# jan-van-bergen/GPU-Raytracer

Hardware: AMD Instinct MI355X
Metric: Mrays/s (primary+secondary) + ms/frame, Sponza 1920x1080 4spp BVH8 (higher is better)
Workload: dtype f32

## Files before the change

### gpu-raytracer_amd/csrc/kernels_trace.hip

```cpp
#include "rt_math.h"

#include <cstdio>
#include <cstdlib>

#ifndef RT_LDS_STACK
#define RT_LDS_STACK   10
#endif
#define RT_STACK_SIZE  32
#define RT_TRACE_BLOCK 256
#ifndef RT_TRACE_WAVES_PER_SIMD
#define RT_TRACE_WAVES_PER_SIMD 6
#endif
#ifndef RT_TRI_BATCH
#define RT_TRI_BATCH 2
#endif
#ifndef RT_FETCH_BLOCK_MAX
#define RT_FETCH_BLOCK_MAX 256
#endif
#ifndef RT_ENDGAME
#define RT_ENDGAME 1
#endif
#ifndef RT_ENDGAME_REGION_MAX
#define RT_ENDGAME_REGION_MAX 256
#endif
// ... 297 lines not shown
}

RT_DEV int opacity_wrap(int i, int n) { if ((n & (n - 1)) == 0) return i & (n - 1); int r = i % n; return r < 0 ? r + n : r; }
RT_DEV bool opacity_accepts(const RtParams & p, int instance, int triangle_id, float u, float v) {
	if (p.has_triangle_aliases) {
		float4 names = p.triangle_positions[size_t(triangle_id) * 3 + 2];
		if (__float_as_int(names.z) >= 0) { instance = __float_as_int(names.z); triangle_id = __float_as_int(names.w); }
	}
	int material = p.mesh_material_ids[instance];
	if (material < 0) return true;
	int mask_index = p.material_opacity[material];
	if (mask_index == RT_INVALID) return true;
	RtOpacityMask mask = p.opacity_masks[mask_index];
	const float4 * shading = p.triangles + size_t(triangle_id) * 6;
	float4 a = shading[4], b = shading[5];
	float s = a.z + u * b.x + v * b.z;
	float t = a.w + u * b.y + v * b.w;
	int x = opacity_wrap(int(floorf(s * float(mask.width))),  mask.width);
	int y = opacity_wrap(int(floorf(t * float(mask.height))), mask.height);
	unsigned i = unsigned(y) * unsigned(mask.width) + unsigned(x);
	return (mask.bits[i >> 5] >> (i & 31u)) & 1u;
}

template<bool MASK = false>
RT_DEV bool triangle_test_kind(bool shadow, float4 part_0, float4 part_1, float4 part_2, int mesh_id, int triangle_id, const Ray3 & ray, HitRecord & hit, const RtParams * p = nullptr) {
	f3 p0 = mk3(part_0.x, part_0.y, part_0.z);
	f3 e1 = mk3(part_0.w, part_1.x, part_1.y);
	f3 e2 = mk3(part_1.z, part_1.w, part_2.x);

	f3 h = cross_fma(ray.direction, e2);
	float a = dot_fma(e1, h);
	float f = 1.0f / a;
	f3 s = ray.origin - p0;
	float u = f * dot_fma(s, h);
	if (u >= 0.0f && u <= 1.0f) {
		f3 q = cross_fma(s, e1);
		float v = f * dot_fma(ray.direction, q);
		if (v >= 0.0f && u + v <= 1.0f) {
			float t = f * dot_fma(e2, q);
			if (t > 0.0f && t < hit.t) {
				if (MASK && !opacity_accepts(*p, mesh_id, triangle_id, u, v)) return false;
				if (shadow) return true;
				hit.t = t; hit.u = u; hit.v = v;
				hit.mesh_id = mesh_id;
				hit.triangle_id = triangle_id;
			}
		}
	}
	return false;
}

template<bool SHADOW>
RT_DEV bool triangle_test(const float4 * __restrict__ triangle_positions, int mesh_id, int triangle_id, const Ray3 & ray, float max_distance, HitRecord & hit) {
	const float4 * tri = triangle_positions + size_t(triangle_id) * 3;
	return triangle_test_loaded<SHADOW>(tri[0], tri[1], tri[2], mesh_id, triangle_id, ray, max_distance, hit);
}

typedef __attribute__((address_space(3))) uint2 LdsUint2;
typedef __attribute__((address_space(1))) uint2 GlobalUint2;
struct TraversalStack {
	LdsUint2    * lds;
	GlobalUint2 * spill;
	int spill_stride;
	int size;

	RT_DEV void push(uint2 item) {
		if (size < RT_LDS_STACK) { lds[size * RT_WAVE_SIZE].x = item.x; lds[size * RT_WAVE_SIZE].y = item.y; }
		else { GlobalUint2 * slot = spill + size_t(size - RT_LDS_STACK) * spill_stride; slot->x = item.x; slot->y = item.y; }
		size++;
	}
	RT_DEV uint2 pop() {
		size--;
		if (size < RT_LDS_STACK) return make_uint2(lds[size * RT_WAVE_SIZE].x, lds[size * RT_WAVE_SIZE].y);
		const GlobalUint2 * slot = spill + size_t(size - RT_LDS_STACK) * spill_stride;
		return make_uint2(slot->x, slot->y);
	}
};


__shared__ uint2 shared_stack[(RT_TRACE_BLOCK / RT_WAVE_SIZE) * RT_LDS_STACK * RT_WAVE_SIZE];
__shared__ int   shared_fetch[RT_TRACE_BLOCK / RT_WAVE_SIZE][4];
#define RT_ROOTS_IN_LDS 1024
__shared__ int   shared_roots[RT_ROOTS_IN_LDS];
enum { RT_TRACE_CLOSEST = 0, RT_TRACE_SHADOW = 1, RT_TRACE_MIXED = 2 };
template<int MODE, typename Source> RT_DEV void source_load(const Source & src, bool shadow, int i, Ray3 & ray, float & max_distance) {
	if constexpr (MODE == RT_TRACE_MIXED) src.load(shadow, i, ray, max_distance); else src.load(i, ray, max_distance);
}
template<int MODE, typename Source> RT_DEV void source_finish(const Source & src, bool shadow, int i, const HitRecord & hit, bool occluded) {
	if constexpr (MODE == RT_TRACE_MIXED) src.finish(shadow, i, hit, occluded); else src.finish(i, hit, occluded);
}

template<int MODE, bool COUNT, bool NARROW, bool UNIFIED = false, bool FLAT = false, bool SKIP = false, bool MASK = false, typename Source>
RT_DEV void bvh8_trace_engine(const RtParams & p, Source & src, int ray_count, int * cursor, unsigned long long * stats = nullptr, int ray_count_2 = 0, int * cursor_2 = nullptr, int * regions = nullptr) {
	constexpr bool SHADOW = MODE == RT_TRACE_SHADOW;
	bool lane_shadow = SHADOW;
	#define RT_IS_SHADOW (MODE == RT_TRACE_MIXED ? lane_shadow : SHADOW)
	const float4 * __restrict__ nodes     = p.bvh8_nodes;
	const float4 * __restrict__ triangles = p.triangle_positions;

	unsigned lane = threadIdx.x & (RT_WAVE_SIZE - 1);
	unsigned wave = threadIdx.x / RT_WAVE_SIZE;
	const unsigned group_child = lane & 7u;
	const unsigned group_base  = lane & ~7u;

	TraversalStack stack;
	stack.lds   = (LdsUint2 *)&shared_stack[wave * (RT_LDS_STACK * RT_WAVE_SIZE) + lane];
	stack.spill_stride = int(gridDim.x * blockDim.x);
	stack.spill = (GlobalUint2 *)(p.stack_spill + (blockIdx.x * blockDim.x + threadIdx.x));
	stack.size  = 0;

	const int waves_in_grid = int(gridDim.x) * (RT_TRACE_BLOCK / RT_WAVE_SIZE);
	const int rays_total = ray_count + (MODE == RT_TRACE_MIXED ? ray_count_2 : 0);
	const bool endgame = !NARROW && regions != nullptr && waves_in_grid <= RT_ENDGAME_MAX_WAVES;
	const int ray_block = NARROW ? 8 : endgame ? RT_FETCH_BLOCK_MAX : max(RT_WAVE_SIZE, min(RT_FETCH_BLOCK_MAX, (rays_total / (RT_FETCH_BLOCK_DIVISOR * waves_in_grid)) & ~(RT_WAVE_SIZE - 1)));
	const int region_size  = max(RT_WAVE_SIZE, min(RT_ENDGAME_REGION_MAX, ((rays_total + waves_in_grid - 1) / waves_in_grid + RT_WAVE_SIZE - 1) & ~(RT_WAVE_SIZE - 1)));
	const int region_count = min(waves_in_grid, (rays_total + region_size - 1) / region_size);
	const int main_limit   = endgame ? max(0, rays_total - region_count * region_size) : 0;
	const int region_stride = max(1, region_count / RT_WAVE_SIZE) | 1;
	const unsigned wave_in_grid = blockIdx.x * (RT_TRACE_BLOCK / RT_WAVE_SIZE) + wave;
	if (endgame ? wave_in_grid >= unsigned(region_count) : wave_in_grid * unsigned(ray_block) >= unsigned(rays_total)) return;
	typedef volatile __attribute__((address_space(3))) int LdsFetchWord;
	LdsFetchWord * fetch_state = (LdsFetchWord *)&shared_fetch[wave][0];
	if (lane == 0) { fetch_state[0] = 0; fetch_state[1] = 0; fetch_state[2] = 0; fetch_state[3] = 0; }
	auto fetch_ray = [&]() -> int {
		while (endgame) {
			if (fetch_state[2]) return -1;
			unsigned long long want = __ballot(1);
			int n_want = __popcll(want);
			unsigned rank = __builtin_amdgcn_mbcnt_hi(unsigned(want >> 32), __builtin_amdgcn_mbcnt_lo(unsigned(want), 0u));
			bool elected = rank == 0;
			int next = fetch_state[0], end = fetch_state[1];
			if (next >= end) {
				int region = fetch_state[3];
				if (region == 0) {
					int base = main_limit;
					if (main_limit > 0) { if (elected) base = atomicAdd(cursor, ray_block); base = __builtin_amdgcn_readfirstlane(base); }
					if (base < main_limit) { next = base; end = min(base + ray_block, main_limit); }
					else region = int(wave_in_grid) + 1;
				}
				if (region != 0) {
					next = 0; end = 0;
					int scan_from = region, scanned = 0;
					while (true) {
						int taken = 0;
						if (elected) taken = atomicAdd(&regions[region - 1], RT_WAVE_SIZE);
						taken = __builtin_amdgcn_readfirstlane(taken);
						int first = main_limit + (region - 1) * region_size + taken;
						if (taken < region_size && first < rays_total) { next = first; end = min(first + RT_WAVE_SIZE, rays_total); break; }
						bool found = false;
						while (!found && scanned < RT_ENDGAME_SCAN_LIMIT) {
							int candidate = scan_from + (int(rank) + 1) * region_stride;
							while (candidate >= region_count) candidate -= region_count;
							int seen = __hip_atomic_load(&regions[candidate], __ATOMIC_RELAXED, __HIP_MEMORY_SCOPE_AGENT);
							bool open = seen < region_size && main_limit + candidate * region_size + seen < rays_total;
							unsigned long long open_lanes = __ballot(open);
							if (open_lanes) {
								int lane_of_first = __ffsll((long long)open_lanes) - 1;
								region = __builtin_amdgcn_readlane(candidate, lane_of_first) + 1; found = true;
							} else { scan_from = scan_from + 1 < region_count ? scan_from + 1 : 0; scanned++; }
						}
						if (!found) break;
					}
				}
				if (elected) fetch_state[3] = region;
			}
			int give = min(n_want, end - next);
			if (elected) {
				fetch_state[0] = next + give;
				fetch_state[1] = end;
				if (next >= end) fetch_state[2] = 1;
			}
			if (int(rank) < give) {
				int index = next + int(rank);
				if (MODE == RT_TRACE_MIXED) { lane_shadow = index >= ray_count; if (lane_shadow) index -= ray_count; }
				return index;
			}
		}
		while (true) {
			if (fetch_state[2]) return -1;
			const bool second_queue = MODE == RT_TRACE_MIXED && fetch_state[3] != 0;
			const int queue_count = second_queue ? ray_count_2 : ray_count;
			int * const queue_cursor = second_queue ? cursor_2 : cursor;
			unsigned long long want = __ballot(1);
			unsigned long long askers = NARROW ? (want & 0x0101010101010101ull) : want;
			int n_want = __popcll(askers);
			bool elected = __builtin_amdgcn_mbcnt_hi(unsigned(want >> 32), __builtin_amdgcn_mbcnt_lo(unsigned(want), 0u)) == 0;
			unsigned rank = NARROW ? unsigned(__popcll(askers & ((1ull << group_base) - 1ull)))
			                       : __builtin_amdgcn_mbcnt_hi(unsigned(want >> 32), __builtin_amdgcn_mbcnt_lo(unsigned(want), 0u));
			int next = fetch_state[0], end = fetch_state[1];
			if (next >= end) {
				int base = 0;
				if (elected) base = atomicAdd(queue_cursor, ray_block);
				base = __builtin_amdgcn_readfirstlane(base);
				next = min(base, queue_count);
				end  = min(base + ray_block, queue_count);
			}
			int give = min(n_want, end - next);
			if (elected) {
				fetch_state[0] = next + give;
				fetch_state[1] = end;
				if (next >= end) {
					if (MODE == RT_TRACE_MIXED && !second_queue) { fetch_state[0] = 0; fetch_state[1] = 0; fetch_state[3] = 1; }
					else fetch_state[2] = 1;
				}
			}
			if (int(rank) < give) { if (MODE == RT_TRACE_MIXED) lane_shadow = second_queue; return next + int(rank); }
		}
	};

	uint2 current_group = make_uint2(0, 0);
	uint2 triangle_group = make_uint2(0, 0);

	int  ray_index = 0;
	Ray3 ray;
	f3   inv_dir;
	unsigned oct_inv4 = 0;
	HitRecord hit;
	int  tlas_stack_size = RT_INVALID;
	int  mesh_id = 0;
	bool mesh_has_identity_transform = true;
	unsigned count_nodes = 0, count_triangles = 0, count_inst_xform = 0, count_inst_ident = 0;

	unsigned long long lane_totals[2][5] = { { 0, 0, 0, 0, 0 }, { 0, 0, 0, 0, 0 } };
	auto flush_counts = [&]() {
		#pragma unroll
		for (int kind = 0; kind < (MODE == RT_TRACE_MIXED ? 2 : 1); kind++) {
			#pragma unroll
			for (int k = 0; k < 5; k++) if (lane_totals[kind][k]) atomicAdd(&stats[kind * 5 + k], lane_totals[kind][k]);
		}
	};
	int result_pending = 0;
	while (true) {
		bool inactive = stack.size == 0 && current_group.y == 0 && triangle_group.y == 0;

		if (result_pending) {
			if (!RT_IS_SHADOW && p.has_triangle_aliases && hit.triangle_id != RT_INVALID) {
				float4 names = triangles[size_t(hit.triangle_id) * 3 + 2];
				if (__float_as_int(names.z) >= 0) { hit.mesh_id = __float_as_int(names.z); hit.triangle_id = __float_as_int(names.w); }
			}
			if (!NARROW || group_child == 0) source_finish<MODE>(src, RT_IS_SHADOW, ray_index, hit, result_pending == 2);
			result_pending = 0;
		}
		if (inactive) {
			ray_index = fetch_ray();
			if (ray_index < 0) { if constexpr (COUNT) flush_counts(); return; }

			float max_distance;
			source_load<MODE>(src, RT_IS_SHADOW, ray_index, ray, max_distance);
			inv_dir  = reciprocal(ray.direction);
			oct_inv4 = ray_get_octant_inv4(ray.direction);

			hit.t = max_distance; hit.u = 0.0f; hit.v = 0.0f; hit.mesh_id = 0; hit.triangle_id = RT_INVALID;
			current_group   = make_uint2(0, 0x80000000u);
			tlas_stack_size = FLAT ? 0 : p.entry_tlas_stack_size;
		}

		int iterations_lost = 0;
		bool running = true;
		do {
			if (running) {
			if (!FLAT && triangle_group.y != 0 && tlas_stack_size == RT_INVALID) {
				int mesh_offset = int(msb(triangle_group.y));
				triangle_group.y &= ~(1u << mesh_offset);
				mesh_id = int(triangle_group.x) + mesh_offset;

				if (triangle_group.y != 0)         stack.push(triangle_group);
				if (current_group.y & 0xff000000u) stack.push(current_group);
				tlas_stack_size = stack.size;
				triangle_group.y = 0;

				unsigned root = unsigned(UNIFIED && p.mesh_count <= RT_ROOTS_IN_LDS ? shared_roots[mesh_id] : p.mesh_bvh_root_indices[mesh_id]);
				mesh_has_identity_transform = (root >> 31) != 0;
				if (!mesh_has_identity_transform) {
					const float4 * m = p.mesh_transforms_inv + size_t(mesh_id) * 3;
					ray.origin    = transform_position (m, ray.origin);
					ray.direction = transform_direction(m, ray.direction);
					inv_dir  = reciprocal(ray.direction);
					oct_inv4 = ray_get_octant_inv4(ray.direction);
					if (COUNT) count_inst_xform++;
				} else if (COUNT) count_inst_ident++;
				current_group = make_uint2(root & 0x7fffffffu, 0x80000000u);
			}

			RT_SETPRIO(RT_PHASE_TOP);
			if (triangle_group.y == 0) {
				if (current_group.y & 0xff000000u) {
					unsigned hits_imask = current_group.y;
					unsigned child_index_offset = msb(hits_imask);
					unsigned child_index_base   = current_group.x;

					current_group.y &= ~(1u << child_index_offset);
					if (current_group.y & 0xff000000u) stack.push(current_group);

					unsigned slot_index     = (child_index_offset - 24) ^ (oct_inv4 & 0xffu);
					unsigned relative_index = __popc(hits_imask & ~(0xffffffffu << slot_index));
					unsigned child_node_index = child_index_base + relative_index;

					const float4 * node = FLAT ? (const float4 *)((const char *)nodes + __umul24(child_node_index, 80u))
					                    : (!UNIFIED && child_node_index < unsigned(p.tlas_node_count) ? p.tlas_nodes : nodes) + size_t(child_node_index) * 5;
					float4 n0 = node[0], n1 = node[1], n2 = node[2], n3 = node[3], n4 = node[4];
					RT_SETPRIO(RT_PHASE_NODE_TEST);
					if (COUNT) count_nodes++;
					unsigned hitmask, bound_bits = 0;
					if (NARROW) {
						int key;
						hitmask = group8_or(bvh8_node_intersect_child(ray, inv_dir, oct_inv4, hit.t, n0, n1, n2, n3, n4, group_child, SKIP ? &key : nullptr));
						if (SKIP) {
							int least = group8_min_signed(key);
							int second = group8_min_signed(key == least ? RT_SKIP_NO_KEY : key);
							bound_bits = skip_bound_bits(hitmask, least, second);
						}
					} else if (RT_FAST_NODE && UNIFIED && FLAT) hitmask = bvh8_node_intersect_fast<SKIP>(ray, inv_dir, oct_inv4, hit.t, n0, n1, n2, n3, n4, &bound_bits);
					else hitmask = bvh8_node_intersect<SKIP>(ray, inv_dir, oct_inv4, hit.t, n0, n1, n2, n3, n4, &bound_bits);
					unsigned imask = extract_byte(__float_as_uint(n0.w), 3);

					current_group .x = __float_as_uint(n1.x);
					triangle_group.x = __float_as_uint(n1.y);
					current_group .y = (hitmask & 0xff000000u) | imask | (SKIP ? bound_bits : 0u);
					triangle_group.y = (hitmask & 0x00ffffffu);
				}
			}
			RT_SETPRIO(RT_PHASE_TRI_ADDRESS);

			bool occluded = false;
			{
				bool has_triangles = triangle_group.y != 0 && (FLAT || tlas_stack_size != RT_INVALID);
				if (has_triangles) {
					if (NARROW) {
						unsigned rest = triangle_group.y; int my_bit = -1;
						#pragma unroll
						for (unsigned k = 0; k < 8; k++) {
							if (rest != 0) { int b = int(msb(rest)); if (k == group_child) my_bit = b; rest &= ~(1u << b); }
						}
						triangle_group.y = rest;
						float t = 0.0f, u = 0.0f, v = 0.0f; bool valid = false; int my_triangle = RT_INVALID;
						if (my_bit >= 0) {
							my_triangle = int(triangle_group.x) + my_bit;
							const float4 * tri = triangles + size_t(my_triangle) * 3;
// ... 68 lines not shown
						oct_inv4 = ray_get_octant_inv4(ray.direction);
					}
				}
				current_group = stack.pop();
				if ((current_group.y & 0xff000000u) == 0) {
					triangle_group = current_group;
					current_group  = make_uint2(0, 0);
				}
				}
			}
			if constexpr (COUNT) if (result_pending) {
				const int kind = MODE == RT_TRACE_MIXED && lane_shadow ? 1 : 0;
				lane_totals[kind][0] += count_nodes;      lane_totals[kind][1] += count_triangles;
				lane_totals[kind][2] += count_inst_xform; lane_totals[kind][3] += count_inst_ident;
				lane_totals[kind][4] += 1;
				count_nodes = count_triangles = count_inst_xform = count_inst_ident = 0;
			}
			}

			iterations_lost += RT_WAVE_SIZE - __popcll(__ballot(running)) - RT_N_D;
		} while (iterations_lost < RT_N_W);
	}
	#undef RT_IS_SHADOW
}


#define RT_TRACE_LAUNCH_WAVES RT_TRACE_WAVES_PER_SIMD
#ifndef RT_MIXED_MAX_RAYS
#define RT_MIXED_MAX_RAYS (10 * 1024 * 1024)
#endif
#ifndef RT_NARROW_MAX_RAYS
#define RT_NARROW_MAX_RAYS 16384
#endif

template<bool SHADOW, bool COUNT, bool MASK = false, typename Source>
RT_DEV void bvh8_trace_persistent(const RtParams & p, const Source & src, int ray_count, int * cursor, unsigned long long * stats = nullptr, bool coherent = false) {
	const bool narrow = !COUNT && !coherent && ray_count <= RT_NARROW_MAX_RAYS;
	if (!SHADOW && rt_skip_walk(p)) {
		if (narrow) bvh8_trace_engine<RT_TRACE_CLOSEST, false, true, false, false, true, MASK>(p, src, ray_count, cursor);
		else bvh8_trace_engine<RT_TRACE_CLOSEST, COUNT, false, false, false, true, MASK>(p, src, ray_count, cursor, stats);
		return;
	}
	if (narrow) bvh8_trace_engine<SHADOW ? RT_TRACE_SHADOW : RT_TRACE_CLOSEST, false, true, false, false, false, MASK>(p, src, ray_count, cursor);
	else bvh8_trace_engine<SHADOW ? RT_TRACE_SHADOW : RT_TRACE_CLOSEST, COUNT, false, false, false, false, MASK>(p, src, ray_count, cursor, stats);
}

RT_DEV uint4 pack_hit(const HitRecord & h) {
	unsigned uv = unsigned(int(h.u * 65535.0f)) | (unsigned(int(h.v * 65535.0f)) << 16);
	return make_uint4(unsigned(h.mesh_id), unsigned(h.triangle_id), __float_as_uint(h.t), uv);
}


struct ClosestHitSource {
	RtVec3SoA origin, direction;
	uint4 * hits;
	RT_DEV void load(int i, Ray3 & ray, float & max_distance) const { ray.origin = load3(origin, i); ray.direction = load3(direction, i); max_distance = RT_INFINITY; }
	RT_DEV void finish(int i, const HitRecord & hit, bool) const { hits[i] = pack_hit(hit); }
};

struct ShadowQueueSource {
	RtShadowBuffer buffer;
	RtAOV radiance, direct, indirect;
	int bounce;
	RT_DEV void load(int i, Ray3 & ray, float & max_distance) const { ray.origin = load3(buffer.origin, i); ray.direction = load3(buffer.direction, i); max_distance = buffer.max_distance[i]; }
	RT_DEV void finish(int i, const HitRecord &, bool occluded) const {
		if (occluded) return;
		float4 ip = buffer.illumination_and_pixel_index[i];
		int pixel_index = __float_as_int(ip.w);
		float4 value = make_float4(ip.x, ip.y, ip.z, 0.0f);
		if (radiance.framebuffer) { float4 c = radiance.framebuffer[pixel_index]; radiance.framebuffer[pixel_index] = make_float4(c.x + value.x, c.y + value.y, c.z + value.z, c.w + value.w); }
		if (bounce == 0) {
			if (direct.framebuffer) direct.framebuffer[pixel_index] = value;
		} else if (indirect.framebuffer) {
			float4 c = indirect.framebuffer[pixel_index];
			indirect.framebuffer[pixel_index] = make_float4(c.x + value.x, c.y + value.y, c.z + value.z, c.w + value.w);
		}
	}
};

struct ShadowStreamSource {
	RtShadowBuffer buffer;
	RtAOV radiance, direct, indirect;
	RT_DEV void load(int i, Ray3 & ray, float & max_distance) const { ray.origin = load3(buffer.origin, i); ray.direction = load3(buffer.direction, i); max_distance = buffer.max_distance[i]; }
	RT_DEV void finish(int i, const HitRecord &, bool occluded) const {
		if (occluded) return;
		float4 ip = buffer.illumination_and_pixel_index[i];
		unsigned pixel_word = __float_as_uint(ip.w);
		int pixel_index = int(pixel_word & ~RT_SHADOW_FLAG_BOUNCE_0);
		float4 value = make_float4(ip.x, ip.y, ip.z, 0.0f);
		if (radiance.framebuffer) { float4 c = radiance.framebuffer[pixel_index]; radiance.framebuffer[pixel_index] = make_float4(c.x + value.x, c.y + value.y, c.z + value.z, c.w + value.w); }
		if (pixel_word & RT_SHADOW_FLAG_BOUNCE_0) {
			if (direct.framebuffer) direct.framebuffer[pixel_index] = value;
		} else if (indirect.framebuffer) {
			float4 c = indirect.framebuffer[pixel_index];
			indirect.framebuffer[pixel_index] = make_float4(c.x + value.x, c.y + value.y, c.z + value.z, c.w + value.w);
		}
	}
};

struct ShadowAOSource {
	RtShadowBuffer buffer;
	RtAOV radiance;
	RT_DEV void load(int i, Ray3 & ray, float & max_distance) const { ray.origin = load3(buffer.origin, i); ray.direction = load3(buffer.direction, i); max_distance = buffer.max_distance[i]; }
	RT_DEV void finish(int i, const HitRecord &, bool occluded) const {
		if (occluded || !radiance.framebuffer) return;
		int pixel_index = __float_as_int(buffer.illumination_and_pixel_index[i].w);
		radiance.framebuffer[pixel_index] = make_float4(1.0f, 1.0f, 1.0f, 1.0f);
	}
};

struct ShadowExplicitSource {
	RtVec3SoA origin, direction;
	const float * max_dist;
	uint8_t * occluded_out;
	RT_DEV void load(int i, Ray3 & ray, float & max_distance) const { ray.origin = load3(origin, i); ray.direction = load3(direction, i); max_distance = max_dist[i]; }
	RT_DEV void finish(int i, const HitRecord &, bool occluded) const { occluded_out[i] = occluded ? 1 : 0; }
};



RT_DEV bool aabb_intersect(f3 lo, f3 hi, const Ray3 & ray, f3 inv_dir, float limit, float & t_near) {
	float t0x = (lo.x - ray.origin.x) * inv_dir.x, t1x = (hi.x - ray.origin.x) * inv_dir.x;
	float t0y = (lo.y - ray.origin.y) * inv_dir.y, t1y = (hi.y - ray.origin.y) * inv_dir.y;
	float t0z = (lo.z - ray.origin.z) * inv_dir.z, t1z = (hi.z - ray.origin.z) * inv_dir.z;
	t_near      = fmaxf(fminf(t0x, t1x), fmaxf(fminf(t0y, t1y), fmaxf(fminf(t0z, t1z), 0.0f)));
	float t_far = fminf(fmaxf(t0x, t1x), fminf(fmaxf(t0y, t1y), fminf(fmaxf(t0z, t1z), limit)));
	return t_near < t_far;
}

struct LeafRange { int first, count; };

struct Bvh2Step {
	const float4 * __restrict__ nodes;
	RT_DEV explicit Bvh2Step(const RtParams & p) : nodes(p.bvh2_nodes) {}
	RT_DEV LeafRange step(const RtParams & p, TraversalStack & stack, uint2 entry, Ray3 ray, f3 inv_dir, float limit) const {
		const float4 * node = (entry.x < unsigned(p.tlas_node_count) ? p.tlas_nodes : nodes) + size_t(entry.x) * 2;
		float4 a = node[0], b = node[1];
		int      left_or_first = __float_as_int(b.z);
		unsigned count_axis    = __float_as_uint(b.w);
		unsigned count = count_axis & 0x3fffffffu, axis = count_axis >> 30;
		float t_near;
		if (!aabb_intersect(mk3(a.x, a.y, a.z), mk3(a.w, b.x, b.y), ray, inv_dir, limit, t_near)) return { 0, 0 };
		if (count > 0) return { left_or_first, int(count) };
		float d = axis == 0 ? ray.direction.x : (axis == 1 ? ray.direction.y : ray.direction.z);
		bool left_first = d > 0.0f;
		stack.push(make_uint2(unsigned(left_first ? left_or_first + 1 : left_or_first), 0));
		stack.push(make_uint2(unsigned(left_first ? left_or_first : left_or_first + 1), 0));
		return { 0, 0 };
	}
};

RT_DEV float float4_at(float4 v, int i) { return i == 0 ? v.x : (i == 1 ? v.y : (i == 2 ? v.z : v.w)); }
struct Bvh4Step {
	const float4 * __restrict__ nodes;
	RT_DEV explicit Bvh4Step(const RtParams & p) : nodes(p.bvh4_nodes) {}
	RT_DEV LeafRange step(const RtParams & p, TraversalStack & stack, uint2 entry, Ray3 ray, f3 inv_dir, float limit) const {
		int index = int(entry.x), count = int(entry.y);
		if (count > 0) return { index, count };
		const float4 * node = (index < p.tlas_node_count ? p.tlas_nodes : nodes) + size_t(index) * 8;
		float4 min_x = node[0], min_y = node[1], min_z = node[2], max_x = node[3], max_y = node[4], max_z = node[5], ic01 = node[6], ic23 = node[7];
		float t_near[4]; unsigned hit_mask = 0;
		#pragma unroll
		for (int i = 0; i < 4; i++) {
			float tn;
			if (aabb_intersect(mk3(float4_at(min_x, i), float4_at(min_y, i), float4_at(min_z, i)),
			                   mk3(float4_at(max_x, i), float4_at(max_y, i), float4_at(max_z, i)), ray, inv_dir, limit, tn)) hit_mask |= 1u << i;
			t_near[i] = __uint_as_float((__float_as_uint(tn) & 0xfffffffcu) | unsigned(i));
		}
// ... 90 lines not shown
					if (tri_next < tri_end && !occluded) {
						const float4 * tri = triangles + size_t(tri_next) * 3;
						if (triangle_test_loaded<SHADOW>(tri[0], tri[1], make_float4(tri[2].x, 0.0f, 0.0f, 0.0f), mesh_id, tri_next, ray, max_distance, hit)) occluded = true;
						tri_next++;
					}
				}
			} else {
				if (stack.size == tlas_stack_size) {
					tlas_stack_size = RT_INVALID;
					if (!mesh_has_identity_transform) {
						float unused;
						src.load(ray_index, ray, unused);
						inv_dir = reciprocal(ray.direction);
					}
				}
				uint2 entry = stack.pop();
				LeafRange leaf = node_step.step(p, stack, entry, ray, inv_dir, SHADOW ? max_distance : hit.t);
				if (leaf.count > 0) {
					if (tlas_stack_size == RT_INVALID) {
						tlas_stack_size = stack.size;
						mesh_id = leaf.first;
						unsigned root = unsigned(p.mesh_bvh_root_indices[mesh_id]);
						mesh_has_identity_transform = (root >> 31) != 0;
						if (!mesh_has_identity_transform) {
							const float4 * m = p.mesh_transforms_inv + size_t(mesh_id) * 3;
							ray.origin    = transform_position (m, ray.origin);
							ray.direction = transform_direction(m, ray.direction);
							inv_dir = reciprocal(ray.direction);
						}
						stack.push(make_uint2(root & 0x7fffffffu, 0));
					} else {
						tri_next = leaf.first; tri_end = leaf.first + leaf.count;
					}
				}
			}

			if (SHADOW && occluded) {
				src.finish(ray_index, hit, true);
				stack.size = 0; tri_next = tri_end = 0;
				break;
			}
			if (stack.size == 0 && tri_next >= tri_end) {
				src.finish(ray_index, hit, false);
				break;
			}
			iterations_lost += RT_WAVE_SIZE - __popcll(__ballot(1)) - RT_N_D;
		} while (iterations_lost < RT_N_W);
	}
}

RT_DEV ClosestHitSource  closest_queue(const RtParams & p, int bounce) { return { p.trace[bounce & 1].origin, p.trace[bounce & 1].direction, p.trace[bounce & 1].hits }; }
RT_DEV ShadowQueueSource shadow_queue (const RtParams & p, int bounce) { return { p.shadow, p.aovs[RT_AOV_RADIANCE], p.aovs[RT_AOV_RADIANCE_DIRECT], p.aovs[RT_AOV_RADIANCE_INDIRECT], bounce }; }
RT_DEV ShadowAOSource    ao_queue     (const RtParams & p)             { return { p.shadow, p.aovs[RT_AOV_RADIANCE] }; }

#ifndef RT_MASK_WAVES
#define RT_MASK_WAVES RT_TRACE_LAUNCH_WAVES
#endif
#define RT_BVH8_KERNELS(SUFFIX, WAVES, MASK) \
__global__ void __launch_bounds__(RT_TRACE_BLOCK, WAVES) kernel_trace_bvh8##SUFFIX(RtParams p, int bounce) { bvh8_trace_persistent<false, false, MASK>(p, closest_queue(p, bounce), p.sizes->trace[bounce], p.ray_cursors + 2 * bounce, nullptr, bounce == 0); } \
__global__ void __launch_bounds__(RT_TRACE_BLOCK, WAVES) kernel_trace_shadow_bvh8##SUFFIX(RtParams p, int bounce) { bvh8_trace_persistent<true, false, MASK>(p, shadow_queue(p, bounce), p.sizes->shadow[bounce], p.ray_cursors + 2 * bounce + 1); } \
__global__ void __launch_bounds__(RT_TRACE_BLOCK, WAVES) kernel_trace_shadow_bvh8_ao##SUFFIX(RtParams p) { bvh8_trace_persistent<true, false, MASK>(p, ao_queue(p), p.sizes->shadow[0], p.ray_cursors + 1); } \
__global__ void __launch_bounds__(RT_TRACE_BLOCK, WAVES) kernel_trace_bvh8_counting##SUFFIX(RtParams p, int bounce, unsigned long long * stats) { bvh8_trace_persistent<false, true, MASK>(p, closest_queue(p, bounce), p.sizes->trace[bounce], p.ray_cursors + 2 * bounce, stats); } \
__global__ void __launch_bounds__(RT_TRACE_BLOCK, WAVES) kernel_trace_shadow_bvh8_counting##SUFFIX(RtParams p, int bounce, unsigned long long * stats) { bvh8_trace_persistent<true, true, MASK>(p, shadow_queue(p, bounce), p.sizes->shadow[bounce], p.ray_cursors + 2 * bounce + 1, stats + 5); } \
__global__ void __launch_bounds__(RT_TRACE_BLOCK, WAVES) kernel_trace_bvh8_explicit##SUFFIX(RtParams p, RtVec3SoA origin, RtVec3SoA direction, uint4 * hits, int ray_count, int * retired) { bvh8_trace_persistent<false, false, MASK>(p, ClosestHitSource { origin, direction, hits }, ray_count, retired); } \
__global__ void __launch_bounds__(RT_TRACE_BLOCK, WAVES) kernel_trace_shadow_bvh8_explicit##SUFFIX(RtParams p, RtVec3SoA origin, RtVec3SoA direction, const float * max_distance, uint8_t * occluded, int ray_count, int * retired) { bvh8_trace_persistent<true, false, MASK>(p, ShadowExplicitSource { origin, direction, max_distance, occluded }, ray_count, retired); }
RT_BVH8_KERNELS(, RT_TRACE_LAUNCH_WAVES, false)
RT_BVH8_KERNELS(_mask, RT_MASK_WAVES, true)
#undef RT_BVH8_KERNELS

#define RT_BVH_KERNELS(WIDTH, STEP) \
__global__ void __launch_bounds__(RT_TRACE_BLOCK, RT_TRACE_LAUNCH_WAVES) kernel_trace_##WIDTH(RtParams p, int bounce) { bvh_trace_persistent<STEP, false>(p, closest_queue(p, bounce), p.sizes->trace[bounce], p.ray_cursors + 2 * bounce); } \
__global__ void __launch_bounds__(RT_TRACE_BLOCK, RT_TRACE_LAUNCH_WAVES) kernel_trace_shadow_##WIDTH(RtParams p, int bounce) { bvh_trace_persistent<STEP, true>(p, shadow_queue(p, bounce), p.sizes->shadow[bounce], p.ray_cursors + 2 * bounce + 1); } \
__global__ void __launch_bounds__(RT_TRACE_BLOCK, RT_TRACE_LAUNCH_WAVES) kernel_trace_shadow_##WIDTH##_ao(RtParams p) { bvh_trace_persistent<STEP, true>(p, ao_queue(p), p.sizes->shadow[0], p.ray_cursors + 1); } \
__global__ void __launch_bounds__(RT_TRACE_BLOCK, RT_TRACE_LAUNCH_WAVES) kernel_trace_##WIDTH##_explicit(RtParams p, RtVec3SoA origin, RtVec3SoA direction, uint4 * hits, int ray_count, int * retired) { bvh_trace_persistent<STEP, false>(p, ClosestHitSource { origin, direction, hits }, ray_count, retired); } \
__global__ void __launch_bounds__(RT_TRACE_BLOCK, RT_TRACE_LAUNCH_WAVES) kernel_trace_shadow_##WIDTH##_explicit(RtParams p, RtVec3SoA origin, RtVec3SoA direction, const float * max_distance, uint8_t * occluded, int ray_count, int * retired) { bvh_trace_persistent<STEP, true>(p, ShadowExplicitSource { origin, direction, max_distance, occluded }, ray_count, retired); }
RT_BVH_KERNELS(bvh2, Bvh2Step)
RT_BVH_KERNELS(bvh4, Bvh4Step)
#undef RT_BVH_KERNELS

struct MixedStreamSource {
	ClosestHitSource closest; ShadowStreamSource shadow;
	RT_DEV void load(bool is_shadow, int i, Ray3 & ray, float & max_distance) const { if (is_shadow) shadow.load(i, ray, max_distance); else closest.load(i, ray, max_distance); }
	RT_DEV void finish(bool is_shadow, int i, const HitRecord & hit, bool occluded) const { if (is_shadow) shadow.finish(i, hit, occluded); else closest.finish(i, hit, occluded); }
};
#ifdef RT_WAVE_CLOCK
#define RT_WAVE_CLOCK_SLOTS 32
#define RT_WAVE_CLOCK_WAVES 16384
__device__ unsigned long long grt_wave_clock[RT_WAVE_CLOCK_SLOTS][RT_WAVE_CLOCK_WAVES][3];
__device__ int grt_wave_clock_meta[RT_WAVE_CLOCK_SLOTS][4];
extern "C" int rt_debug_read_wave_clock(void * clocks, void * meta) {
	if (hipMemcpyFromSymbol(clocks, HIP_SYMBOL(grt_wave_clock), sizeof(grt_wave_clock)) != hipSuccess) return 1;
	return hipMemcpyFromSymbol(meta, HIP_SYMBOL(grt_wave_clock_meta), sizeof(grt_wave_clock_meta)) != hipSuccess;
}
template<bool COUNT, bool FLAT = false, bool SKIP = false, bool MASK = false> RT_DEV void trace_stream_probed(const RtParams & p, unsigned long long * stats, unsigned long long * mid);
template<bool COUNT, bool FLAT = false, bool SKIP = false, bool MASK = false>
RT_DEV void trace_stream(const RtParams & p, unsigned long long * stats) {
	const unsigned long long t0 = __builtin_amdgcn_s_memrealtime();
	unsigned long long t1 = 0;
	trace_stream_probed<COUNT, FLAT, SKIP, MASK>(p, stats, &t1);
	const unsigned long long t2 = __builtin_amdgcn_s_memrealtime();
	if ((threadIdx.x & 63) == 0) {
		const int slot = p.stream_iteration % RT_WAVE_CLOCK_SLOTS, wave = blockIdx.x * (RT_TRACE_BLOCK / RT_WAVE_SIZE) + threadIdx.x / RT_WAVE_SIZE;
		if (wave < RT_WAVE_CLOCK_WAVES) { grt_wave_clock[slot][wave][0] = t0; grt_wave_clock[slot][wave][1] = t1 ? t1 : t2; grt_wave_clock[slot][wave][2] = t2; }
		if (wave == 0) { const int q = p.stream_iteration & 1; grt_wave_clock_meta[slot][0] = p.stream_iteration; grt_wave_clock_meta[slot][1] = p.stream->trace_count[q]; grt_wave_clock_meta[slot][2] = p.stream->shadow_count[q ^ 1]; grt_wave_clock_meta[slot][3] = gridDim.x * (RT_TRACE_BLOCK / RT_WAVE_SIZE); }
	}
}
#define trace_stream_body trace_stream_probed
#define RT_WAVE_CLOCK_MID , unsigned long long * mid
#define RT_WAVE_CLOCK_MARK *mid = __builtin_amdgcn_s_memrealtime();
#else
template<bool COUNT, bool FLAT = false, bool SKIP = false, bool MASK = false> RT_DEV void trace_stream(const RtParams & p, unsigned long long * stats);
#define trace_stream_body trace_stream
#define RT_WAVE_CLOCK_MID
#define RT_WAVE_CLOCK_MARK
#endif
template<bool COUNT, bool FLAT, bool SKIP, bool MASK>
RT_DEV void trace_stream_body(const RtParams & p, unsigned long long * stats RT_WAVE_CLOCK_MID) {
	const int q = p.stream_iteration & 1;
	MixedStreamSource src { { p.trace[q].origin, p.trace[q].direction, p.trace[q].hits },
	                        { p.shadow, p.aovs[RT_AOV_RADIANCE], p.aovs[RT_AOV_RADIANCE_DIRECT], p.aovs[RT_AOV_RADIANCE_INDIRECT] } };
	const int closest_count = p.stream->trace_count[q], shadow_count = p.stream->shadow_count[q ^ 1];
	if (!FLAT && p.mesh_count <= RT_ROOTS_IN_LDS) {
		for (int i = threadIdx.x; i < p.mesh_count; i += RT_TRACE_BLOCK) shared_roots[i] = p.mesh_bvh_root_indices[i];
		__syncthreads();
	}
	if (!COUNT && closest_count + shadow_count <= RT_NARROW_MAX_RAYS)
		bvh8_trace_engine<RT_TRACE_MIXED, false, true, true, FLAT, SKIP, MASK>(p, src, closest_count, &p.stream->cursor[q][0], nullptr, shadow_count, &p.stream->cursor[q][1]);
	else if (COUNT || closest_count + shadow_count <= RT_MIXED_MAX_RAYS)
		bvh8_trace_engine<RT_TRACE_MIXED, COUNT, false, true, FLAT, SKIP, MASK>(p, src, closest_count, &p.stream->cursor[q][0], stats, shadow_count, &p.stream->cursor[q][1], RT_ENDGAME ? &p.stream->endgame[q][0][0] : nullptr);
	else {
		bvh8_trace_engine<RT_TRACE_CLOSEST, false, false, true, FLAT, SKIP, MASK>(p, src.closest, closest_count, &p.stream->cursor[q][0], nullptr, 0, nullptr, RT_ENDGAME ? &p.stream->endgame[q][0][0] : nullptr);
		RT_WAVE_CLOCK_MARK
		bvh8_trace_engine<RT_TRACE_SHADOW,  false, false, true, FLAT, false, MASK>(p, src.shadow,  shadow_count,  &p.stream->cursor[q][1], nullptr, 0, nullptr, RT_ENDGAME ? &p.stream->endgame[q][1][0] : nullptr);
	}
}
__global__ void __launch_bounds__(RT_TRACE_BLOCK, RT_TRACE_LAUNCH_WAVES) kernel_trace_stream_bvh8(RtParams p) { trace_stream<false>(p, nullptr); }
#ifndef RT_FLAT_WAVES
#define RT_FLAT_WAVES (RT_FAST_NODE ? 6 : 7)
#endif
__global__ void __launch_bounds__(RT_TRACE_BLOCK, RT_FLAT_WAVES) kernel_trace_stream_bvh8_flat(RtParams p) { trace_stream<false, true>(p, nullptr); }
#ifndef RT_FLAT_SKIP_WAVES
#define RT_FLAT_SKIP_WAVES RT_FLAT_WAVES
#endif
__global__ void __launch_bounds__(RT_TRACE_BLOCK, RT_FLAT_SKIP_WAVES) kernel_trace_stream_bvh8_flat_skip(RtParams p) { trace_stream<false, true, true>(p, nullptr); }
__global__ void __launch_bounds__(RT_TRACE_BLOCK, RT_TRACE_LAUNCH_WAVES) kernel_trace_stream_bvh8_counting(RtParams p, unsigned long long * stats) {
	if (rt_skip_walk(p)) trace_stream<true, false, true>(p, stats); else trace_stream<true>(p, stats);
}
__global__ void __launch_bounds__(RT_TRACE_BLOCK, RT_MASK_WAVES) kernel_trace_stream_bvh8_mask(RtParams p) { trace_stream<false, false, false, true>(p, nullptr); }
__global__ void __launch_bounds__(RT_TRACE_BLOCK, RT_MASK_WAVES) kernel_trace_stream_bvh8_flat_mask(RtParams p) { trace_stream<false, true, false, true>(p, nullptr); }
__global__ void __launch_bounds__(RT_TRACE_BLOCK, RT_MASK_WAVES) kernel_trace_stream_bvh8_flat_skip_mask(RtParams p) { trace_stream<false, true, true, true>(p, nullptr); }
__global__ void __launch_bounds__(RT_TRACE_BLOCK, RT_MASK_WAVES) kernel_trace_stream_bvh8_counting_mask(RtParams p, unsigned long long * stats) {
	if (rt_skip_walk(p)) trace_stream<true, false, true, true>(p, stats); else trace_stream<true, false, false, true>(p, stats);
}

static int trace_grid_size(const void * kernel) {
	static const int cus = [] {
		int device = 0, count = 0;
		(void)hipGetDevice(&device);
		(void)hipDeviceGetAttribute(&count, hipDeviceAttributeMultiprocessorCount, device);
		return count > 0 ? count : 256;
	}();
	int blocks_per_cu = 0;
	if (hipOccupancyMaxActiveBlocksPerMultiprocessor(&blocks_per_cu, kernel, RT_TRACE_BLOCK, 0) != hipSuccess || blocks_per_cu <= 0) blocks_per_cu = 2;
	if (blocks_per_cu > 8) blocks_per_cu = 8;
	return cus * blocks_per_cu;
}

template<auto K> static int persistent_grid() {
	static const int grid = trace_grid_size((const void *)K);
	return grid;
}
template<auto K, typename... A> static void launch_persistent(hipStream_t stream, const A &... args) {
	hipLaunchKernelGGL(K, dim3(persistent_grid<K>()), dim3(RT_TRACE_BLOCK), 0, stream, args...);
}
template<auto K8, auto K8M, typename... A> static void launch_for_mask(const RtParams & p, hipStream_t stream, const A &... args) {
	if (p.opacity_active) launch_persistent<K8M>(stream, p, args...);
	else launch_persistent<K8>(stream, p, args...);
}
template<auto K2, auto K4, auto K8, auto K8M, typename... A> static void launch_for_width(const RtParams & p, hipStream_t stream, const A &... args) {
	if (p.bvh_width == 2) launch_persistent<K2>(stream, p, args...);
	else if (p.bvh_width == 4) launch_persistent<K4>(stream, p, args...);
	else launch_for_mask<K8, K8M>(p, stream, args...);
}

void rt_launch_trace(const RtParams & p, int bounce, hipStream_t stream) {
	launch_for_width<kernel_trace_bvh2, kernel_trace_bvh4, kernel_trace_bvh8, kernel_trace_bvh8_mask>(p, stream, bounce);
}
void rt_launch_trace_shadow(const RtParams & p, int bounce, hipStream_t stream) {
	launch_for_width<kernel_trace_shadow_bvh2, kernel_trace_shadow_bvh4, kernel_trace_shadow_bvh8, kernel_trace_shadow_bvh8_mask>(p, stream, bounce);
}
void rt_launch_trace_shadow_ao(const RtParams & p, hipStream_t stream) {
	launch_for_width<kernel_trace_shadow_bvh2_ao, kernel_trace_shadow_bvh4_ao, kernel_trace_shadow_bvh8_ao, kernel_trace_shadow_bvh8_ao_mask>(p, stream);
}
static int stream_kernel_id(const RtParams & p, bool stats) {
	const int kernel = stats ? RT_STREAM_KERNEL_COUNTING
	                 : p.entry_tlas_stack_size == 0 && p.geometry_below_4gib ? (rt_skip_walk(p) ? RT_STREAM_KERNEL_FLAT_SKIP : RT_STREAM_KERNEL_FLAT)
	                 : RT_STREAM_KERNEL_GENERAL;
	return p.opacity_active ? kernel + RT_STREAM_KERNEL_GENERAL_MASK : kernel;
}
struct StreamKernel { void (*launch)(hipStream_t, const RtParams &, unsigned long long *); int (*grid)(); };
template<auto K> static void launch_stream(hipStream_t stream, const RtParams & p, unsigned long long *) { launch_persistent<K>(stream, p); }
template<auto K> static void launch_stream_counting(hipStream_t stream, const RtParams & p, unsigned long long * stats) { launch_persistent<K>(stream, p, stats); }
static const StreamKernel stream_kernels[] = {
	{ launch_stream<kernel_trace_stream_bvh8>,                        persistent_grid<kernel_trace_stream_bvh8> },
	{ launch_stream<kernel_trace_stream_bvh8_flat>,                   persistent_grid<kernel_trace_stream_bvh8_flat> },
	{ launch_stream<kernel_trace_stream_bvh8_flat_skip>,              persistent_grid<kernel_trace_stream_bvh8_flat_skip> },
	{ launch_stream_counting<kernel_trace_stream_bvh8_counting>,      persistent_grid<kernel_trace_stream_bvh8_counting> },
	{ launch_stream<kernel_trace_stream_bvh8_mask>,                   persistent_grid<kernel_trace_stream_bvh8_mask> },
	{ launch_stream<kernel_trace_stream_bvh8_flat_mask>,              persistent_grid<kernel_trace_stream_bvh8_flat_mask> },
	{ launch_stream<kernel_trace_stream_bvh8_flat_skip_mask>,         persistent_grid<kernel_trace_stream_bvh8_flat_skip_mask> },
	{ launch_stream_counting<kernel_trace_stream_bvh8_counting_mask>, persistent_grid<kernel_trace_stream_bvh8_counting_mask> },
};
static_assert(RT_STREAM_KERNEL_GENERAL == 0 && RT_STREAM_KERNEL_FLAT == 1 && RT_STREAM_KERNEL_FLAT_SKIP == 2 && RT_STREAM_KERNEL_COUNTING == 3 &&
              RT_STREAM_KERNEL_GENERAL_MASK == 4 && RT_STREAM_KERNEL_FLAT_MASK == 5 && RT_STREAM_KERNEL_FLAT_SKIP_MASK == 6 && RT_STREAM_KERNEL_COUNTING_MASK == 7 &&
              sizeof(stream_kernels) / sizeof(stream_kernels[0]) == 8, "stream_kernels is indexed by RT_STREAM_KERNEL_*");
void rt_launch_trace_stream(const RtParams & p, unsigned long long * stats, hipStream_t stream) {
// ... 19 lines not shown
```

Baseline: 3954.

## Defer unoccluded shadow-ray contributions into a per-wave LDS list and flush in batches

Shadow rays that finish unoccluded no longer write their radiance contribution inline. Their ray indices are appended to a per-wave LDS list, which is flushed cooperatively across all live lanes once it holds a full wave's worth of entries, and again on exit. The aim is to avoid the divergent, serialized global accumulation that happens when only a few lanes finish at once, so accumulation runs wave-wide. The cost is extra LDS use per wave, ballot and bookkeeping on every loop iteration, and an occasional flush stall. Refill-timing probe instrumentation under RT_WAVE_CLOCK is also added.

```diff
diff --git a/gpu-raytracer_amd/csrc/kernels_trace.hip b/gpu-raytracer_amd/csrc/kernels_trace.hip
--- a/gpu-raytracer_amd/csrc/kernels_trace.hip
+++ b/gpu-raytracer_amd/csrc/kernels_trace.hip
@@ -403,6 +403,13 @@
 __shared__ int   shared_fetch[RT_TRACE_BLOCK / RT_WAVE_SIZE][4];
 #define RT_ROOTS_IN_LDS 1024
 __shared__ int   shared_roots[RT_ROOTS_IN_LDS];
+#ifndef RT_SHADOW_BATCH
+#define RT_SHADOW_BATCH 1
+#endif
+#define RT_CONTRIBUTION_LIST (2 * RT_WAVE_SIZE)
+__shared__ int   shared_fetch_and_contributions[RT_TRACE_BLOCK / RT_WAVE_SIZE][8 + RT_CONTRIBUTION_LIST];
+template<typename Source, typename = void> struct source_defers_contributions { static constexpr bool value = false; };
+template<typename Source> struct source_defers_contributions<Source, decltype(void(&Source::contribute))> { static constexpr bool value = RT_SHADOW_BATCH != 0; };
 enum { RT_TRACE_CLOSEST = 0, RT_TRACE_SHADOW = 1, RT_TRACE_MIXED = 2 };
 template<int MODE, typename Source> RT_DEV void source_load(const Source & src, bool shadow, int i, Ray3 & ray, float & max_distance) {
 	if constexpr (MODE == RT_TRACE_MIXED) src.load(shadow, i, ray, max_distance); else src.load(i, ray, max_distance);
@@ -411,9 +418,29 @@
 	if constexpr (MODE == RT_TRACE_MIXED) src.finish(shadow, i, hit, occluded); else src.finish(i, hit, occluded);
 }
 
+#ifdef RT_WAVE_CLOCK
+#define RT_REFILL_PROBE_PARAMETER , unsigned * refill_probe = nullptr
+#define RT_REFILL_PROBE_ENTER const unsigned long long probe_entered = __builtin_amdgcn_s_memrealtime(); unsigned long long probe_begin = probe_entered; unsigned probe_ticks = 0, probe_refills = 0, probe_handover = 0;
+#define RT_REFILL_PROBE_BEGIN __builtin_amdgcn_sched_barrier(0); probe_begin = __builtin_amdgcn_s_memrealtime(); __builtin_amdgcn_sched_barrier(0);
+#define RT_REFILL_PROBE_MID   __builtin_amdgcn_sched_barrier(0); probe_handover += unsigned(__builtin_amdgcn_s_memrealtime() - probe_begin); __builtin_amdgcn_sched_barrier(0);
+#define RT_REFILL_PROBE_END   __builtin_amdgcn_sched_barrier(0); __builtin_amdgcn_s_waitcnt(0x0070);  \
+	probe_ticks += unsigned(__builtin_amdgcn_s_memrealtime() - probe_begin); probe_refills++; __builtin_amdgcn_sched_barrier(0);
+#define RT_REFILL_PROBE_LEAVE if (refill_probe) { const unsigned long long probe_now = __builtin_amdgcn_s_memrealtime(); \
+	refill_probe[0] = probe_ticks + unsigned(probe_now - probe_begin); refill_probe[1] = probe_refills + 1; refill_probe[2] = unsigned(probe_now - probe_entered); refill_probe[3] = probe_handover; }
+#else
+#define RT_REFILL_PROBE_PARAMETER
+#define RT_REFILL_PROBE_ENTER
+#define RT_REFILL_PROBE_BEGIN
+#define RT_REFILL_PROBE_MID
+#define RT_REFILL_PROBE_END
+#define RT_REFILL_PROBE_LEAVE
+#endif
+
 template<int MODE, bool COUNT, bool NARROW, bool UNIFIED = false, bool FLAT = false, bool SKIP = false, bool MASK = false, typename Source>
-RT_DEV void bvh8_trace_engine(const RtParams & p, Source & src, int ray_count, int * cursor, unsigned long long * stats = nullptr, int ray_count_2 = 0, int * cursor_2 = nullptr, int * regions = nullptr) {
+RT_DEV void bvh8_trace_engine(const RtParams & p, Source & src, int ray_count, int * cursor, unsigned long long * stats = nullptr, int ray_count_2 = 0, int * cursor_2 = nullptr, int * regions = nullptr RT_REFILL_PROBE_PARAMETER) {
+	RT_REFILL_PROBE_ENTER
 	constexpr bool SHADOW = MODE == RT_TRACE_SHADOW;
+	constexpr bool DEFER = MODE != RT_TRACE_CLOSEST && source_defers_contributions<Source>::value;
 	bool lane_shadow = SHADOW;
 	#define RT_IS_SHADOW (MODE == RT_TRACE_MIXED ? lane_shadow : SHADOW)
 	const float4 * __restrict__ nodes     = p.bvh8_nodes;
@@ -441,8 +468,18 @@
 	const unsigned wave_in_grid = blockIdx.x * (RT_TRACE_BLOCK / RT_WAVE_SIZE) + wave;
 	if (endgame ? wave_in_grid >= unsigned(region_count) : wave_in_grid * unsigned(ray_block) >= unsigned(rays_total)) return;
 	typedef volatile __attribute__((address_space(3))) int LdsFetchWord;
-	LdsFetchWord * fetch_state = (LdsFetchWord *)&shared_fetch[wave][0];
+	LdsFetchWord * fetch_state = DEFER ? (LdsFetchWord *)&shared_fetch_and_contributions[wave][0] : (LdsFetchWord *)&shared_fetch[wave][0];
 	if (lane == 0) { fetch_state[0] = 0; fetch_state[1] = 0; fetch_state[2] = 0; fetch_state[3] = 0; }
+	LdsFetchWord * contribution_count = fetch_state + 4;
+	if (DEFER && lane == 0) contribution_count[0] = 0;
+	auto contribution_flush = [&](int held) {
+		if constexpr (DEFER) {
+			const unsigned long long live = __ballot(1);
+			const int step = __popcll(live);
+			LdsFetchWord * contribution_list = fetch_state; asm volatile("" : "+v"(contribution_list)); contribution_list += 8;
+			for (int entry = int(__builtin_amdgcn_mbcnt_hi(unsigned(live >> 32), __builtin_amdgcn_mbcnt_lo(unsigned(live), 0u))); entry < held; entry += step) src.contribute(contribution_list[entry]);
+		}
+	};
 	auto fetch_ray = [&]() -> int {
 		while (endgame) {
 			if (fetch_state[2]) return -1;
@@ -552,8 +589,23 @@
 	};
 	int result_pending = 0;
 	while (true) {
+		RT_REFILL_PROBE_BEGIN
 		bool inactive = stack.size == 0 && current_group.y == 0 && triangle_group.y == 0;
 
+		if constexpr (DEFER) {
+			const bool append = RT_IS_SHADOW && result_pending == 1 && (!NARROW || group_child == 0);
+			const unsigned long long appenders = __ballot(append);
+			if (appenders) {
+				int held = contribution_count[0];
+				if (held >= RT_WAVE_SIZE) { contribution_flush(held); held = 0; }
+				const unsigned rank = __builtin_amdgcn_mbcnt_hi(unsigned(appenders >> 32), __builtin_amdgcn_mbcnt_lo(unsigned(appenders), 0u));
+				if (append) {
+					fetch_state[8 + held + int(rank)] = ray_index;
+					if (rank == 0) contribution_count[0] = held + __popcll(appenders);
+				}
+			}
+			if (RT_IS_SHADOW) result_pending = 0;
+		}
 		if (result_pending) {
 			if (!RT_IS_SHADOW && p.has_triangle_aliases && hit.triangle_id != RT_INVALID) {
 				float4 names = triangles[size_t(hit.triangle_id) * 3 + 2];
@@ -562,9 +614,15 @@
 			if (!NARROW || group_child == 0) source_finish<MODE>(src, RT_IS_SHADOW, ray_index, hit, result_pending == 2);
 			result_pending = 0;
 		}
+		RT_REFILL_PROBE_MID
 		if (inactive) {
 			ray_index = fetch_ray();
-			if (ray_index < 0) { if constexpr (COUNT) flush_counts(); return; }
+			if (ray_index < 0) {
+				if constexpr (DEFER) { const int held = contribution_count[0]; if (held) { contribution_flush(held); contribution_count[0] = 0; } }
+				if constexpr (COUNT) flush_counts();
+				RT_REFILL_PROBE_LEAVE
+				return;
+			}
 
 			float max_distance;
 			source_load<MODE>(src, RT_IS_SHADOW, ray_index, ray, max_distance);
@@ -575,6 +633,7 @@
 			current_group   = make_uint2(0, 0x80000000u);
 			tlas_stack_size = FLAT ? 0 : p.entry_tlas_stack_size;
 		}
+		RT_REFILL_PROBE_END
 
 		int iterations_lost = 0;
 		bool running = true;
@@ -809,8 +868,8 @@
 	RtShadowBuffer buffer;
 	RtAOV radiance, direct, indirect;
 	RT_DEV void load(int i, Ray3 & ray, float & max_distance) const { ray.origin = load3(buffer.origin, i); ray.direction = load3(buffer.direction, i); max_distance = buffer.max_distance[i]; }
-	RT_DEV void finish(int i, const HitRecord &, bool occluded) const {
-		if (occluded) return;
+	RT_DEV void finish(int i, const HitRecord &, bool occluded) const { if (!occluded) contribute(i); }
+	RT_DEV void contribute(int i) const {
 		float4 ip = buffer.illumination_and_pixel_index[i];
 		unsigned pixel_word = __float_as_uint(ip.w);
 		int pixel_index = int(pixel_word & ~RT_SHADOW_FLAG_BOUNCE_0);
@@ -1067,6 +1126,7 @@
 	ClosestHitSource closest; ShadowStreamSource shadow;
 	RT_DEV void load(bool is_shadow, int i, Ray3 & ray, float & max_distance) const { if (is_shadow) shadow.load(i, ray, max_distance); else closest.load(i, ray, max_distance); }
 	RT_DEV void finish(bool is_shadow, int i, const HitRecord & hit, bool occluded) const { if (is_shadow) shadow.finish(i, hit, occluded); else closest.finish(i, hit, occluded); }
+	RT_DEV void contribute(int i) const { shadow.contribute(i); }
 };
 #ifdef RT_WAVE_CLOCK
 #define RT_WAVE_CLOCK_SLOTS 32
@@ -1077,27 +1137,41 @@
 	if (hipMemcpyFromSymbol(clocks, HIP_SYMBOL(grt_wave_clock), sizeof(grt_wave_clock)) != hipSuccess) return 1;
 	return hipMemcpyFromSymbol(meta, HIP_SYMBOL(grt_wave_clock_meta), sizeof(grt_wave_clock_meta)) != hipSuccess;
 }
-template<bool COUNT, bool FLAT = false, bool SKIP = false, bool MASK = false> RT_DEV void trace_stream_probed(const RtParams & p, unsigned long long * stats, unsigned long long * mid);
+__device__ unsigned grt_refill_clock[RT_WAVE_CLOCK_SLOTS][RT_WAVE_CLOCK_WAVES][3][4];
+extern "C" int rt_debug_read_refill_clock(void * ticks) {
+	return hipMemcpyFromSymbol(ticks, HIP_SYMBOL(grt_refill_clock), sizeof(grt_refill_clock)) != hipSuccess;
+}
+template<bool COUNT, bool FLAT = false, bool SKIP = false, bool MASK = false> RT_DEV void trace_stream_probed(const RtParams & p, unsigned long long * stats, unsigned long long * mid, unsigned (* refill)[4]);
 template<bool COUNT, bool FLAT = false, bool SKIP = false, bool MASK = false>
 RT_DEV void trace_stream(const RtParams & p, unsigned long long * stats) {
 	const unsigned long long t0 = __builtin_amdgcn_s_memrealtime();
 	unsigned long long t1 = 0;
-	trace_stream_probed<COUNT, FLAT, SKIP, MASK>(p, stats, &t1);
+	unsigned refill[3][4] = { { 0, 0, 0, 0 }, { 0, 0, 0, 0 }, { 0, 0, 0, 0 } };
+	trace_stream_probed<COUNT, FLAT, SKIP, MASK>(p, stats, &t1, refill);
 	const unsigned long long t2 = __builtin_amdgcn_s_memrealtime();
+	#pragma unroll
+	for (int k = 0; k < 12; k++) {
+		unsigned v = refill[k / 4][k % 4];
+		for (int offset = RT_WAVE_SIZE / 2; offset > 0; offset >>= 1) v = max(v, unsigned(__shfl_xor(int(v), offset)));
+		refill[k / 4][k % 4] = v;
+	}
 	if ((threadIdx.x & 63) == 0) {
 		const int slot = p.stream_iteration % RT_WAVE_CLOCK_SLOTS, wave = blockIdx.x * (RT_TRACE_BLOCK / RT_WAVE_SIZE) + threadIdx.x / RT_WAVE_SIZE;
+		if (wave < RT_WAVE_CLOCK_WAVES) for (int k = 0; k < 12; k++) grt_refill_clock[slot][wave][k / 4][k % 4] = refill[k / 4][k % 4];
 		if (wave < RT_WAVE_CLOCK_WAVES) { grt_wave_clock[slot][wave][0] = t0; grt_wave_clock[slot][wave][1] = t1 ? t1 : t2; grt_wave_clock[slot][wave][2] = t2; }
 		if (wave == 0) { const int q = p.stream_iteration & 1; grt_wave_clock_meta[slot][0] = p.stream_iteration; grt_wave_clock_meta[slot][1] = p.stream->trace_count[q]; grt_wave_clock_meta[slot][2] = p.stream->shadow_count[q ^ 1]; grt_wave_clock_meta[slot][3] = gridDim.x * (RT_TRACE_BLOCK / RT_WAVE_SIZE); }
 	}
 }
 #define trace_stream_body trace_stream_probed
-#define RT_WAVE_CLOCK_MID , unsigned long long * mid
+#define RT_WAVE_CLOCK_MID , unsigned long long * mid, unsigned (* refill)[4]
+#define RT_REFILL_PROBE_OF(engine) , refill[engine]
 #define RT_WAVE_CLOCK_MARK *mid = __builtin_amdgcn_s_memrealtime();
 #else
 template<bool COUNT, bool FLAT = false, bool SKIP = false, bool MASK = false> RT_DEV void trace_stream(const RtParams & p, unsigned long long * stats);
 #define trace_stream_body trace_stream
 #define RT_WAVE_CLOCK_MID
 #define RT_WAVE_CLOCK_MARK
+#define RT_REFILL_PROBE_OF(engine)
 #endif
 template<bool COUNT, bool FLAT, bool SKIP, bool MASK>
 RT_DEV void trace_stream_body(const RtParams & p, unsigned long long * stats RT_WAVE_CLOCK_MID) {
@@ -1112,11 +1186,11 @@
 	if (!COUNT && closest_count + shadow_count <= RT_NARROW_MAX_RAYS)
 		bvh8_trace_engine<RT_TRACE_MIXED, false, true, true, FLAT, SKIP, MASK>(p, src, closest_count, &p.stream->cursor[q][0], nullptr, shadow_count, &p.stream->cursor[q][1]);
 	else if (COUNT || closest_count + shadow_count <= RT_MIXED_MAX_RAYS)
-		bvh8_trace_engine<RT_TRACE_MIXED, COUNT, false, true, FLAT, SKIP, MASK>(p, src, closest_count, &p.stream->cursor[q][0], stats, shadow_count, &p.stream->cursor[q][1], RT_ENDGAME ? &p.stream->endgame[q][0][0] : nullptr);
+		bvh8_trace_engine<RT_TRACE_MIXED, COUNT, false, true, FLAT, SKIP, MASK>(p, src, closest_count, &p.stream->cursor[q][0], stats, shadow_count, &p.stream->cursor[q][1], RT_ENDGAME ? &p.stream->endgame[q][0][0] : nullptr RT_REFILL_PROBE_OF(2));
 	else {
-		bvh8_trace_engine<RT_TRACE_CLOSEST, false, false, true, FLAT, SKIP, MASK>(p, src.closest, closest_count, &p.stream->cursor[q][0], nullptr, 0, nullptr, RT_ENDGAME ? &p.stream->endgame[q][0][0] : nullptr);
+		bvh8_trace_engine<RT_TRACE_CLOSEST, false, false, true, FLAT, SKIP, MASK>(p, src.closest, closest_count, &p.stream->cursor[q][0], nullptr, 0, nullptr, RT_ENDGAME ? &p.stream->endgame[q][0][0] : nullptr RT_REFILL_PROBE_OF(0));
 		RT_WAVE_CLOCK_MARK
-		bvh8_trace_engine<RT_TRACE_SHADOW,  false, false, true, FLAT, false, MASK>(p, src.shadow,  shadow_count,  &p.stream->cursor[q][1], nullptr, 0, nullptr, RT_ENDGAME ? &p.stream->endgame[q][1][0] : nullptr);
+		bvh8_trace_engine<RT_TRACE_SHADOW,  false, false, true, FLAT, false, MASK>(p, src.shadow,  shadow_count,  &p.stream->cursor[q][1], nullptr, 0, nullptr, RT_ENDGAME ? &p.stream->endgame[q][1][0] : nullptr RT_REFILL_PROBE_OF(1));
 	}
 }
 __global__ void __launch_bounds__(RT_TRACE_BLOCK, RT_TRACE_LAUNCH_WAVES) kernel_trace_stream_bvh8(RtParams p) { trace_stream<false>(p, nullptr); }
```

Result: faster. 3999, median of 6 (+1.1%).
